# entn-at/exemplars_vc

Measured on AMD Instinct MI355X. Metric: spectral frames/sec converted (100 NMF iters, N=4096 dict), higher is better.
Workload: dtype f64

## Files before the change

exemplars_vc_amd/csrc/evc_fused_all.hip:

```cpp
#include "evc_fused_common.h"

namespace evc {

constexpr int AW = 4;
constexpr int AKT = 8;
constexpr int ATILES = AW * AKT;
constexpr int ATHREADS = 2 * AW * 64;
constexpr unsigned ALL_POLL_LIMIT = 1u << 17;
#ifndef EVC_ALL_STAGGER_PER_ITER
#define EVC_ALL_STAGGER_PER_ITER 11000
#endif
#ifndef EVC_ALL_EXCH_PRIO
#define EVC_ALL_EXCH_PRIO 3
#endif
#ifndef EVC_ALL_C1_ALTERNATE
#define EVC_ALL_C1_ALTERNATE 0
#endif

#ifdef EVC_ALL_TIMING
#define EVC_STAMP(i)                                                                                             \
    do {                                                                                                         \
        if (a.dbg && tt0 == g - half && lane == 0 && w == 0)                                                     \
            a.dbg[(((long)blockIdx.x * 2 + half) * (2 * a.iters + 1) + step) * 4 + (i)] = __builtin_amdgcn_s_memtime(); \
    } while (0)
#else
#define EVC_STAMP(i)
#endif

template <int MSTEPS, int C, bool KL>
__global__ __launch_bounds__(ATHREADS, 2) void k_fused_all(FusedArgs a) {
    constexpr int MT = MSTEPS > 4 ? 2 : 1;
    constexpr int E = MT * 4 * 64;
    constexpr int NE = MSTEPS * 64;
    constexpr int MSP = (MSTEPS + 1) & ~1;
    __shared__ double s_red[2][AW * E];
    __shared__ double s_v[2][E];
    __shared__ double s_x[2][E];
    __shared__ double s_r[2][KL ? E : 1];
    __shared__ double s_stage[2][C > 0 ? 1 : 768];
    __shared__ unsigned s_hb[2];
    __shared__ int s_fail;
    const int tid = threadIdx.x, lane = tid & 63;
    const int w8 = __builtin_amdgcn_readfirstlane(tid >> 6);
    const int half = w8 >> 2, w = w8 & 3, th = tid & (AW * 64 - 1);
    const int CR = C > 0 ? C : a.coop_c;
    const int member = blockIdx.x % CR;
    const int g = 2 * (blockIdx.x / CR) + half;
    double* const red = s_red[half];
    double* const vL = s_v[half];
    double* const xL = s_x[half];
    double* const rL = s_r[half];
    double* const stage = s_stage[half];
    unsigned hb = 0;
    const double* __restrict__ A1p = a.A1p;
    const double* __restrict__ A2p = a.A2p;
    f64x2* __restrict__ Hp = a.Hp;
    const int NT = a.NT;
    const long tile0 = (long)member * ATILES + w;
    const unsigned ul = (unsigned)lane;
    long sw = 0;

    const __amdgpu_buffer_rsrc_t r1 = __builtin_amdgcn_make_buffer_rsrc(const_cast<double*>(A1p), 0, NT * (MSP * 512), 0x00020000);
    const __amdgpu_buffer_rsrc_t r2 = __builtin_amdgcn_make_buffer_rsrc(const_cast<double*>(A2p), 0, NT * (MT * 2048), 0x00020000);
#ifdef EVC_ALL_NOFRAG
    bool nofrag_go = false;
#endif
    const unsigned ul16 = ul * 16u, ul8 = ul * 8u;
    auto load_a1 = [&](double (&a1)[MSTEPS], int k) {
#ifdef EVC_ALL_NOFRAG
        if (nofrag_go) return;
#endif
        const int so = (int)(tile0 + sw + AW * k) * (MSP * 512);
#pragma unroll
        for (int s = 0; s < MSTEPS; s += 2) {
            if (s + 1 < MSTEPS) {
                const f64x2 v = __builtin_bit_cast(f64x2, __builtin_amdgcn_raw_buffer_load_b128(r1, ul16 + (s >> 1) * 1024, so, 0));
                a1[s] = v[0];
                a1[s + 1] = v[1];
            } else {
                a1[s] = __builtin_bit_cast(double, __builtin_amdgcn_raw_buffer_load_b64(r1, ul16 + (s >> 1) * 1024, so, 0));
            }
        }
    };
    auto load_a2 = [&](double (&a2)[MT][4], int k) {
#ifdef EVC_ALL_NOFRAG
        if (nofrag_go) return;
#endif
        const int so = (int)(tile0 + sw + AW * k) * (MT * 2048);
#pragma unroll
        for (int u = 0; u < MT; ++u)
#pragma unroll
            for (int r = 0; r < 4; r += 2) {
                const f64x2 v = __builtin_bit_cast(f64x2, __builtin_amdgcn_raw_buffer_load_b128(r2, ul16 + (u * 2 + (r >> 1)) * 1024, so, 0));
                a2[u][r] = v[0];
                a2[u][r + 1] = v[1];
            }
    };
    (void)ul8;

    const int mode = a.eps_mode;
    const double eps = a.eps;
    const double d0 = a.l1 + (mode == EVC_EPS_ADD ? a.eps : 0.0);
    const f64x4 dinit = {d0, d0, d0, d0};
    const unsigned lo = fast_lo(mode, eps);
    unsigned seq = 0;
    int rs_es = 1, rs_len = 0, rs_pub0 = 0, rs_pub1 = 0, rs_src0 = -1, rs_src1 = -1, rs_src2 = -1;
    if (C < 0) {
        rs_es = (NE + CR - 1) / CR;
        rs_len = NE - member * rs_es;
        rs_len = rs_len < 0 ? 0 : (rs_len > rs_es ? rs_es : rs_len);
        const int e0 = th, e1 = th + AW * 64;
        const int j0 = e0 / rs_es, j1 = (e1 < NE ? e1 : e0) / rs_es;
        rs_pub0 = (j0 * CR + member) * rs_es + (e0 - j0 * rs_es);
        rs_pub1 = (j1 * CR + member) * rs_es + ((e1 < NE ? e1 : e0) - j1 * rs_es);
        auto src = [&](int idx) {
            if (idx >= CR * rs_es) return -1;
            const int el = idx % rs_es;
            return el < rs_len ? member * CR * rs_es + idx : -1;
        };
        rs_src0 = src(th);
        rs_src1 = src(th + AW * 64);
        rs_src2 = src(th + 2 * AW * 64);
    }
    if (tid == 0) s_fail = 0;
    if (tid < 2) s_hb[tid] = 0;

    if (a.stagger_cycles > 0 && ((blockIdx.x / CR) & 1)) {
        const long long t0 = __builtin_amdgcn_s_memtime();
        while (__builtin_amdgcn_s_memtime() - t0 < a.stagger_cycles) __builtin_amdgcn_s_sleep(32);
    }

    for (long tt0 = g - half; tt0 < a.TT; tt0 += a.groups) {
        const long tt = tt0 + half;
        bool valid;
        {
            const long t = 16 * tt + (lane & 15);
            int u = -1;
            if (tt < a.TT && t < a.T_) u = a.frame_utt[t];
            const bool live = tt < a.TT && ((t >= a.T_) || ((u >= 0) && (a.active[u] != 0)));
            const int v0 = __syncthreads_and(half == 0 ? live : true);
            const int v1 = __syncthreads_and(half == 1 ? live : true);
            valid = (half ? v1 : v0) != 0;
        }
        HTile h[AKT];
        f64x4 p[AKT];
        double a1[MSTEPS], a2[MT][4];
        if (valid && a.first && a.init_const) {
            auto h0_of = [&](int fr) {
                const long t = 16 * tt + fr;
                const int u = t < a.T_ ? a.frame_utt[t] : -1;
                return u >= 0 ? a.h0[u] : 0.0;
            };
            for (int e = th; e < E; e += AW * 64) {
                const int s = e >> 6, l = e & 63;
                const bool in = s < MSTEPS;
                xL[e] = in ? a.Xp[(tt * MSTEPS + s) * 64 + l] : 0.0;
                vL[e] = in ? a.rsum[bin_of(s, l >> 4)] * h0_of(l & 15) : 0.0;
                if (KL) rL[e] = xL[e] / (vL[e] < a.eps ? a.eps : vL[e]);
            }
            const double hv = h0_of(lane & 15);
#pragma unroll
            for (int k = 0; k < AKT; ++k) {
                const long n0 = 16 * (tile0 + AW * k) + 4 * (lane >> 4);
#pragma unroll
                for (int r = 0; r < 4; ++r) h[k][r] = n0 + r < a.N ? hv : 0.0;
            }
        } else if (valid) {
            for (int e = th; e < E; e += AW * 64) {
                const int s = e >> 6, l = e & 63;
                const bool in = s < MSTEPS;
                xL[e] = in ? a.Xp[(tt * MSTEPS + s) * 64 + l] : 0.0;
                vL[e] = in ? a.Vp[(tt * 8 + s) * 64 + l] : 0.0;
                if (KL) rL[e] = xL[e] / (vL[e] < a.eps ? a.eps : vL[e]);
            }
#pragma unroll
            for (int k = 0; k < AKT; ++k) {
                const f64x2* t = Hp + (tt * NT + tile0 + AW * k) * 128;
                const f64x2 h01 = t[ul], h23 = t[ul + 64];
                h[k][0] = h01[0]; h[k][1] = h01[1]; h[k][2] = h23[0]; h[k][3] = h23[1];
            }
        }
        __syncthreads();
        if (valid && !KL) {
            double x[MSTEPS];
#pragma unroll
            for (int s = 0; s < MSTEPS; ++s) x[s] = xL[s * 64 + lane];
            load_a1(a1, 0);
#pragma unroll
            for (int k = 0; k < AKT; ++k) {
                f64x4 acc = {0, 0, 0, 0};
#pragma unroll
                for (int s = 0; s < MSTEPS; ++s) acc = Mma<double>::mma(a1[s], x[s], acc);
                load_a1(a1, (k + 1) % AKT);
                p[k] = acc;
            }
        }

        if (valid && KL) load_a1(a1, 0);
        for (int step = 0; step <= 2 * a.iters; ++step) {
#ifdef EVC_ALL_NOFRAG
            nofrag_go = step > 2;
#endif
            const bool mine = (C == 1 && !EVC_ALL_C1_ALTERNATE) ? (step & 1) == 0 : (step & 1) == half;
            EVC_STAMP(0);
            if (valid && mine && step < 2 * a.iters) {
                asm volatile("" : "+s"(sw));
                double v[MSTEPS];
#pragma unroll
                for (int s = 0; s < MSTEPS; ++s) v[s] = KL ? rL[s * 64 + lane] : vL[s * 64 + lane];
                f64x4 vn[MT];
#pragma unroll
                for (int u = 0; u < MT; ++u) vn[u] = f64x4{0, 0, 0, 0};
#pragma unroll
                for (int k = 0; k < AKT; ++k) {
                    __builtin_amdgcn_sched_barrier(0);
                    load_a2(a2, k);
                    f64x4 d = KL ? f64x4{0, 0, 0, 0} : dinit;
#pragma unroll
                    for (int s = 0; s < MSTEPS; ++s) d = Mma<double>::mma(a1[s], v[s], d);
                    load_a1(a1, (k + 1) % AKT);
                    __builtin_amdgcn_sched_barrier(0);
                    if (KL) {
#pragma unroll
                        for (int r = 0; r < 4; ++r) h[k][r] *= d[r];
                    } else {
                        mu_tile_guarded(h[k], p[k], d, mode, eps, lo);
                    }
#pragma unroll
                    for (int u = 0; u < MT; ++u)
#pragma unroll
                        for (int r = 0; r < 4; ++r) vn[u] = Mma<double>::mma(a2[u][r], h[k][r], vn[u]);
                }
#pragma unroll
                for (int u = 0; u < MT; ++u)
#pragma unroll
                    for (int r = 0; r < 4; ++r)
                        if (u * 4 + r < MSTEPS) red[w * E + (u * 4 + r) * 64 + lane] = vn[u][r];
            } else if (valid && !mine && step > 0) {
                const int e0 = C <= 0 ? th % NE : th, e1 = th + AW * 64;
                const bool has1 = e1 < NE;
                __builtin_amdgcn_s_setprio(EVC_ALL_EXCH_PRIO);
                double s0 = 0.0, s1 = 0.0;
#pragma unroll
                for (int ww = 0; ww < AW; ++ww) {
                    s0 += red[ww * E + e0];
                    s1 += red[ww * E + (has1 ? e1 : e0)];
                }
                if (C < 0) {
                    long long* xb1 = reinterpret_cast<long long*>(a.coop_buf) +
                                     ((size_t)(seq & 1) * a.groups + g) * (size_t)CR * ALL_RS_STRIDE;
                    long long* xb2 = reinterpret_cast<long long*>(a.coop_buf) + ALL_SLICE_OFFSET +
                                     ((size_t)(seq & 1) * a.groups + g) * 512;
                    const long long tag = (seq >> 1) & 1;
                    __hip_atomic_store(xb1 + rs_pub0, (__double_as_longlong(s0) & ~1LL) | tag, __ATOMIC_RELAXED,
                                       __HIP_MEMORY_SCOPE_AGENT);
                    if (has1)
                        __hip_atomic_store(xb1 + rs_pub1, (__double_as_longlong(s1) & ~1LL) | tag, __ATOMIC_RELAXED,
                                           __HIP_MEMORY_SCOPE_AGENT);
                    bool ok = true;
                    auto fetch3 = [&](const long long* p0, const long long* p1, const long long* p2, long long& b0,
                                      long long& b1, long long& b2) {
                        unsigned polls = 0;
                        for (;;) {
                            b0 = __hip_atomic_load(p0, __ATOMIC_RELAXED, __HIP_MEMORY_SCOPE_AGENT);
                            b1 = __hip_atomic_load(p1, __ATOMIC_RELAXED, __HIP_MEMORY_SCOPE_AGENT);
                            b2 = __hip_atomic_load(p2, __ATOMIC_RELAXED, __HIP_MEMORY_SCOPE_AGENT);
                            if (__all(!ok || (((b0 ^ tag) | (b1 ^ tag) | (b2 ^ tag)) & 1) == 0)) break;
                            if (++polls > ALL_POLL_LIMIT ||
                                ((polls & 63) == 0 &&
                                 __hip_atomic_load(a.coop_abort, __ATOMIC_RELAXED, __HIP_MEMORY_SCOPE_AGENT) != 0))
                                ok = false;
                            __builtin_amdgcn_s_sleep(1);
                        }
                    };
                    {
                        long long b0, b1, b2;
                        const long long* own = xb1 + rs_pub0;
                        fetch3(rs_src0 >= 0 ? xb1 + rs_src0 : own, rs_src1 >= 0 ? xb1 + rs_src1 : own,
                               rs_src2 >= 0 ? xb1 + rs_src2 : own, b0, b1, b2);
                        if (rs_src0 >= 0) stage[th] = __longlong_as_double(b0 & ~1LL);
                        if (rs_src1 >= 0) stage[th + AW * 64] = __longlong_as_double(b1 & ~1LL);
                        if (rs_src2 >= 0) stage[th + 2 * AW * 64] = __longlong_as_double(b2 & ~1LL);
                        hb += AW;
                        if (lane == 0)
                            __hip_atomic_fetch_add(&s_hb[half], 1u, __ATOMIC_RELEASE, __HIP_MEMORY_SCOPE_WORKGROUP);
                        while ((int)(__hip_atomic_load(&s_hb[half], __ATOMIC_ACQUIRE, __HIP_MEMORY_SCOPE_WORKGROUP) - hb) < 0)
                            __builtin_amdgcn_s_sleep(1);
                        const int q = th & 3;
                        for (int el = th >> 2; el < rs_len; el += AW * 16) {
                            double v = 0.0;
                            for (int m = q; m < CR; m += 4) v += stage[m * rs_es + el];
                            v += __shfl_xor(v, 1, 64);
                            v += __shfl_xor(v, 2, 64);
                            if (q == 0)
                                __hip_atomic_store(xb2 + member * rs_es + el, (__double_as_longlong(v) & ~1LL) | tag,
                                                   __ATOMIC_RELAXED, __HIP_MEMORY_SCOPE_AGENT);
                        }
                    }
                    long long g0, g1, g2;
                    fetch3(xb2 + e0, xb2 + (has1 ? e1 : e0), xb2 + e0, g0, g1, g2);
                    s0 = __longlong_as_double(g0 & ~1LL);
                    s1 = __longlong_as_double(g1 & ~1LL);
                    ++seq;
                    if (!ok) s_fail = 1;
                } else if (C == 0) {
                    const int ES = NE / CR;
                    long long* xb1 = reinterpret_cast<long long*>(a.coop_buf) +
                                     ((size_t)(seq & 1) * a.groups + g) * (size_t)CR * 512;
                    long long* xb2 = reinterpret_cast<long long*>(a.coop_buf) + ALL_SLICE_OFFSET +
                                     ((size_t)(seq & 1) * a.groups + g) * 512;
                    const long long tag = (seq >> 1) & 1;
                    {
                        const int j0 = e0 / ES, j1 = (has1 ? e1 : e0) / ES;
                        __hip_atomic_store(xb1 + ((size_t)j0 * CR + member) * ES + (e0 - j0 * ES),
                                           (__double_as_longlong(s0) & ~1LL) | tag, __ATOMIC_RELAXED,
                                           __HIP_MEMORY_SCOPE_AGENT);
                        if (has1)
                            __hip_atomic_store(xb1 + ((size_t)j1 * CR + member) * ES + (e1 - j1 * ES),
                                               (__double_as_longlong(s1) & ~1LL) | tag, __ATOMIC_RELAXED,
                                               __HIP_MEMORY_SCOPE_AGENT);
                    }
                    bool ok = true;
                    auto fetch2 = [&](const long long* p0, const long long* p1, long long& b0, long long& b1) {
                        unsigned polls = 0;
                        for (;;) {
                            b0 = __hip_atomic_load(p0, __ATOMIC_RELAXED, __HIP_MEMORY_SCOPE_AGENT);
                            b1 = __hip_atomic_load(p1, __ATOMIC_RELAXED, __HIP_MEMORY_SCOPE_AGENT);
                            if (__all(!ok || (((b0 ^ tag) | (b1 ^ tag)) & 1) == 0)) break;
                            if (++polls > ALL_POLL_LIMIT ||
                                ((polls & 63) == 0 &&
                                 __hip_atomic_load(a.coop_abort, __ATOMIC_RELAXED, __HIP_MEMORY_SCOPE_AGENT) != 0))
                                ok = false;
                            __builtin_amdgcn_s_sleep(1);
                        }
                    };
                    {
                        long long b0, b1;
                        const long long* mine_ = xb1 + (size_t)member * NE;
                        fetch2(mine_ + e0, mine_ + (has1 ? e1 : e0), b0, b1);
                        stage[e0] = __longlong_as_double(b0 & ~1LL);
                        if (has1) stage[e1] = __longlong_as_double(b1 & ~1LL);
                        hb += AW;
                        if (lane == 0)
                            __hip_atomic_fetch_add(&s_hb[half], 1u, __ATOMIC_RELEASE, __HIP_MEMORY_SCOPE_WORKGROUP);
                        while ((int)(__hip_atomic_load(&s_hb[half], __ATOMIC_ACQUIRE, __HIP_MEMORY_SCOPE_WORKGROUP) - hb) < 0)
                            __builtin_amdgcn_s_sleep(1);
                        if (th < 4 * ES) {
                            const int el = th >> 2, q = th & 3, per = CR >> 2;
                            double v = 0.0;
                            for (int i = 0; i < per; ++i) v += stage[(q * per + i) * ES + el];
                            v += __shfl_xor(v, 1, 64);
                            v += __shfl_xor(v, 2, 64);
                            if (q == 0)
                                __hip_atomic_store(xb2 + member * ES + el, (__double_as_longlong(v) & ~1LL) | tag,
                                                   __ATOMIC_RELAXED, __HIP_MEMORY_SCOPE_AGENT);
                        }
                    }
                    long long g0, g1;
                    fetch2(xb2 + e0, xb2 + (has1 ? e1 : e0), g0, g1);
                    s0 = __longlong_as_double(g0 & ~1LL);
                    s1 = __longlong_as_double(g1 & ~1LL);
                    ++seq;
                    if (!ok) s_fail = 1;
                } else if (C > 1) {
                    long long* xb = reinterpret_cast<long long*>(a.coop_buf) +
                                    ((size_t)(seq & 1) * a.groups + g) * (size_t)(C * 512);
                    const long long tag = (seq >> 1) & 1;
                    const long long m0 = (__double_as_longlong(s0) & ~1LL) | tag;
                    const long long m1 = (__double_as_longlong(s1) & ~1LL) | tag;
                    __hip_atomic_store(xb + member * 512 + e0, m0, __ATOMIC_RELAXED, __HIP_MEMORY_SCOPE_AGENT);
                    if (has1) __hip_atomic_store(xb + member * 512 + e1, m1, __ATOMIC_RELAXED, __HIP_MEMORY_SCOPE_AGENT);
                    bool ok = true;
                    unsigned polls = 0;
                    {
                        const long long* sp = xb + (lane < C ? lane : 0) * 512 + (NE - 1);
                        for (;;) {
                            const long long b = __hip_atomic_load(sp, __ATOMIC_RELAXED, __HIP_MEMORY_SCOPE_AGENT);
                            const bool ready = lane >= C || lane == member || (b & 1) == tag;
                            if (__all(ready)) break;
                            if (++polls > ALL_POLL_LIMIT ||
                                ((polls & 63) == 0 &&
                                 __hip_atomic_load(a.coop_abort, __ATOMIC_RELAXED, __HIP_MEMORY_SCOPE_AGENT) != 0)) {
                                ok = false;
                                break;
                            }
                            __builtin_amdgcn_s_sleep(2);
                        }
                    }
                    long long b0[C > 0 ? C : 1] = {}, b1[C > 0 ? C : 1] = {};
                    polls = 0;
                    while (ok) {
#pragma unroll
                        for (int m = 0; m < C; ++m)
                            b0[m] = __hip_atomic_load(xb + m * 512 + e0, __ATOMIC_RELAXED, __HIP_MEMORY_SCOPE_AGENT);
#pragma unroll
                        for (int m = 0; m < C; ++m)
                            b1[m] = __hip_atomic_load(xb + m * 512 + (has1 ? e1 : e0), __ATOMIC_RELAXED, __HIP_MEMORY_SCOPE_AGENT);
                        long long bad = 0;
#pragma unroll
                        for (int m = 0; m < C; ++m) {
                            b0[m] = (m == member) ? m0 : b0[m];
                            b1[m] = (m == member) ? m1 : b1[m];
                            bad |= (b0[m] ^ tag) | (b1[m] ^ tag);
                        }
                        if ((bad & 1) == 0) break;
                        if (++polls > ALL_POLL_LIMIT ||
                            ((polls & 63) == 0 &&
                             __hip_atomic_load(a.coop_abort, __ATOMIC_RELAXED, __HIP_MEMORY_SCOPE_AGENT) != 0)) {
                            ok = false;
                            break;
                        }
                        __builtin_amdgcn_s_sleep(2);
                    }
                    s0 = 0.0; s1 = 0.0;
#pragma unroll
                    for (int m = 0; m < C; ++m) {
                        s0 += __longlong_as_double(b0[m] & ~1LL);
                        s1 += __longlong_as_double(b1[m] & ~1LL);
                    }
                    ++seq;
                    if (!ok) s_fail = 1;
                }
                vL[e0] = s0;
                if (has1) vL[e1] = s1;
                if (KL) {
                    rL[e0] = xL[e0] / (s0 < a.eps ? a.eps : s0);
                    if (has1) rL[e1] = xL[e1] / (s1 < a.eps ? a.eps : s1);
                }
                __builtin_amdgcn_s_setprio(0);
            }
            EVC_STAMP(1);
            __syncthreads();
            EVC_STAMP(2);
            if (C != 1 && s_fail) {
                if (tid == 0) __hip_atomic_store(a.coop_abort, 1, __ATOMIC_RELAXED, __HIP_MEMORY_SCOPE_AGENT);
                return;
            }
        }

        if (valid) {
#pragma unroll
            for (int k = 0; k < AKT; ++k) {
                f64x2* t = Hp + (tt * NT + tile0 + AW * k) * 128;
                t[ul] = f64x2{h[k][0], h[k][1]};
                t[ul + 64] = f64x2{h[k][2], h[k][3]};
            }
            if (a.Hx) {
                const long t = 16 * tt + (lane & 15);
                if (t < a.T_) {
#pragma unroll
                    for (int k = 0; k < AKT; ++k) {
                        const long n0 = 16 * (tile0 + AW * k) + 4 * (lane >> 4);
#pragma unroll
                        for (int r = 0; r < 4; ++r)
                            if (n0 + r < a.N) {
                                if (a.hx_frame_major) a.Hx[t * a.ldhx + n0 + r] = h[k][r];
                                else a.Hx[(n0 + r) * a.ldhx + t] = h[k][r];
                            }
                    }
                }
            }
            if (member == 0) {
                for (int e = th; e < NE; e += AW * 64) a.Vp[(tt * 8 + (e >> 6)) * 64 + (e & 63)] = vL[e];
                if (a.write_err && w == 0) {
                    double e = 0.0;
#pragma unroll
                    for (int s = 0; s < MSTEPS; ++s) {
                        const double x = xL[s * 64 + lane], vv = vL[s * 64 + lane];
                        e += KL ? kl_terms(x, vv, a.eps) : (x - vv) * (x - vv);
                    }
                    e += __shfl_xor(e, 16, 64);
                    e += __shfl_xor(e, 32, 64);
                    const long t = 16 * tt + lane;
                    if (lane < 16 && t < a.T_) a.err2[t] = e;
                }
            }
        }
        __syncthreads();
    }
}

template <int MSTEPS, int C, bool KL>
static hipError_t launch_all(FusedArgs a, int n_cus, hipStream_t s) {
    int occ = 0;
    hipError_t e = hipOccupancyMaxActiveBlocksPerMultiprocessor(&occ, k_fused_all<MSTEPS, C, KL>, ATHREADS, 0);
    if (e != hipSuccess) return e;
    if (occ < 1) return hipErrorInvalidValue;
    long resident = n_cus;
    if (2 * resident > ALL_MAX_WGS) resident = ALL_MAX_WGS / 2;
    const int cr = C > 0 ? C : a.coop_c;
    if (C == 0 && (cr < 8 || cr > 64 || (cr & (cr - 1)))) return hipErrorInvalidValue;
    if (C < 0 && (cr < 2 || cr > ALL_MAX_MEMBERS)) return hipErrorInvalidValue;
    int pairs = (int)(resident / cr);
    const int want = (a.TT + 1) / 2;
    if (pairs > want) pairs = want;
    if (pairs < 1) return hipErrorInvalidValue;
    a.groups = 2 * pairs;
    a.stagger_cycles = (a.iters > 0 && a.iters <= 25 && a.TT >= 4L * a.groups && pairs >= 2) ? (long long)a.iters * EVC_ALL_STAGGER_PER_ITER : 0;
    if (C != 1) {
        e = hipMemsetAsync(a.coop_buf, 0xFF, sizeof(double) * 2 * (size_t)a.groups * cr * (C < 0 ? ALL_RS_STRIDE : 512), s);
        if (e != hipSuccess) return e;
    }
    if (C <= 0) {
        if (2L * a.groups * 512 > ALL_SLICE_ELEMS) return hipErrorInvalidValue;
        e = hipMemsetAsync(a.coop_buf + ALL_SLICE_OFFSET, 0xFF, sizeof(double) * 2 * (size_t)a.groups * 512, s);
        if (e != hipSuccess) return e;
    }
    hipLaunchKernelGGL((k_fused_all<MSTEPS, C, KL>), dim3((unsigned)(pairs * cr)), dim3(ATHREADS), 0, s, a);
    return hipGetLastError();
}

template <int MSTEPS, bool KL>
static hipError_t pick_c(const FusedArgs& a, int n_cus, hipStream_t s) {
    switch (a.NT / ATILES) {
        case 1: return launch_all<MSTEPS, 1, KL>(a, n_cus, s);
        case 2: return launch_all<MSTEPS, 2, KL>(a, n_cus, s);
        case 4: return launch_all<MSTEPS, 4, KL>(a, n_cus, s);
#ifdef EVC_ALL_DIRECT8
        case 8: return launch_all<MSTEPS, 8, KL>(a, n_cus, s);
#else
        case 8:
#endif
        case 16:
        case 32:
        case 64: return launch_all<MSTEPS, 0, KL>(a, n_cus, s);
        default: return launch_all<MSTEPS, -1, KL>(a, n_cus, s);
    }
}

int fused_all_members(int NT, int N, int eps_mode, int exact_div, int loss) {
    if (eps_mode == EVC_EPS_NONE || exact_div || (loss != EVC_LOSS_FROBENIUS && loss != EVC_LOSS_KL)) return 0;
    if (NT % ATILES) return 0;
    const int c = NT / ATILES;
    if (loss == EVC_LOSS_KL && c >= 2 && c < 16) return 0;
    return (c >= 1 && c <= ALL_MAX_MEMBERS) ? c : 0;
}

hipError_t fused_all_launch(int msteps, const FusedArgs& a, int n_cus, hipStream_t s) {
    if (a.NT % ATILES || !a.coop_buf || !a.coop_abort) return hipErrorInvalidValue;
    switch (msteps) {
        case 1: return a.loss == EVC_LOSS_KL ? pick_c<1, true>(a, n_cus, s) : pick_c<1, false>(a, n_cus, s);
        case 2: return a.loss == EVC_LOSS_KL ? pick_c<2, true>(a, n_cus, s) : pick_c<2, false>(a, n_cus, s);
        case 3: return a.loss == EVC_LOSS_KL ? pick_c<3, true>(a, n_cus, s) : pick_c<3, false>(a, n_cus, s);
        case 4: return a.loss == EVC_LOSS_KL ? pick_c<4, true>(a, n_cus, s) : pick_c<4, false>(a, n_cus, s);
        case 5: return a.loss == EVC_LOSS_KL ? pick_c<5, true>(a, n_cus, s) : pick_c<5, false>(a, n_cus, s);
        case 6: return a.loss == EVC_LOSS_KL ? pick_c<6, true>(a, n_cus, s) : pick_c<6, false>(a, n_cus, s);
        case 7: return a.loss == EVC_LOSS_KL ? pick_c<7, true>(a, n_cus, s) : pick_c<7, false>(a, n_cus, s);
        case 8: return a.loss == EVC_LOSS_KL ? pick_c<8, true>(a, n_cus, s) : pick_c<8, false>(a, n_cus, s);
        default: return hipErrorInvalidValue;
    }
}

}
```

Baseline: 1.052 million.

## Keep each workgroup's dictionary slice resident in LDS instead of reloading from global

When it fits in the LDS budget and the loss is Frobenius, each workgroup copies its dictionary tiles once into shared memory in a padded, row-permuted layout. Both matrix-product phases then read the A1/A2 fragments from LDS instead of issuing buffer loads from global memory on every NMF iteration. The 8-member case is routed to a direct C=8 instantiation when the dictionary fits. This adds LDS pressure, which may lower occupancy, adds a one-time fill cost, and sizes the reduction and staging buffers from compile-time shape constants.

Result: faster. 1.095 million (median of 6 runs) (+4.1%).

```diff
diff --git a/exemplars_vc_amd/csrc/evc_fused_all.hip b/exemplars_vc_amd/csrc/evc_fused_all.hip
--- a/exemplars_vc_amd/csrc/evc_fused_all.hip
+++ b/exemplars_vc_amd/csrc/evc_fused_all.hip
@@ -16,6 +16,25 @@
 #ifndef EVC_ALL_C1_ALTERNATE
 #define EVC_ALL_C1_ALTERNATE 0
 #endif
+
+constexpr long ALL_LDS_BUDGET = 160 * 1024 - 256;
+__host__ __device__ constexpr int all_dict_row(int e) { return 4 * (((e >> 2) & 1) * 2 + (e >> 3)) + (e & 3); }
+template <int MSTEPS, int C, bool KL>
+struct AllShape {
+    static constexpr int MT = MSTEPS > 4 ? 2 : 1;
+    static constexpr int E = MT * 4 * 64;
+    static constexpr int NE = MSTEPS * 64;
+    static constexpr int RSTR = NE < 256 ? 256 : NE;
+    static constexpr int STG = C > 0 ? 1 : (C == 0 ? NE : NE + ALL_MAX_MEMBERS - 1);
+    static constexpr long REST = 8L * 2 * (AW * RSTR + 2 * E + (KL ? E : 1) + STG) + 3 * 4;
+    static constexpr long dict_bytes(int pr) { return 8L * ATILES * 16 * pr; }
+    static constexpr int PR_ALL = 4 * MSTEPS + 2;
+    static constexpr int PR = KL ? 0
+                              : REST + dict_bytes(PR_ALL) <= ALL_LDS_BUDGET       ? PR_ALL
+                              : REST + dict_bytes(PR_ALL - 4) <= ALL_LDS_BUDGET   ? PR_ALL - 4
+                                                                                  : 0;
+    static constexpr bool LDS_DICT = C != 1 && PR > 0 && PR - 1 >= 4 * MSTEPS - 3;
+};
 
 #ifdef EVC_ALL_TIMING
 #define EVC_STAMP(i)                                                                                             \
@@ -29,15 +48,20 @@
 
 template <int MSTEPS, int C, bool KL>
 __global__ __launch_bounds__(ATHREADS, 2) void k_fused_all(FusedArgs a) {
-    constexpr int MT = MSTEPS > 4 ? 2 : 1;
-    constexpr int E = MT * 4 * 64;
-    constexpr int NE = MSTEPS * 64;
+    using S = AllShape<MSTEPS, C, KL>;
+    constexpr int MT = S::MT;
+    constexpr int E = S::E;
+    constexpr int NE = S::NE;
+    constexpr int RSTR = S::RSTR;
     constexpr int MSP = (MSTEPS + 1) & ~1;
-    __shared__ double s_red[2][AW * E];
+    constexpr int PR = S::PR;
+    constexpr int TPD = 16 * PR;
+    __shared__ double s_red[2][AW * RSTR];
     __shared__ double s_v[2][E];
     __shared__ double s_x[2][E];
     __shared__ double s_r[2][KL ? E : 1];
-    __shared__ double s_stage[2][C > 0 ? 1 : 768];
+    __shared__ double s_stage[2][S::STG];
+    __shared__ double s_dict[S::LDS_DICT ? ATILES * TPD : 1];
     __shared__ unsigned s_hb[2];
     __shared__ int s_fail;
     const int tid = threadIdx.x, lane = tid & 63;
@@ -66,7 +90,23 @@
     bool nofrag_go = false;
 #endif
     const unsigned ul16 = ul * 16u, ul8 = ul * 8u;
-    auto load_a1 = [&](double (&a1)[MSTEPS], int k) {
+    constexpr int BL = 16 * ((MSTEPS - 1) >> 2) + 4 * ((MSTEPS - 1) & 3);
+    const int rowA = w * AKT * TPD + all_dict_row(4 * (lane & 3) + ((lane & 15) >> 2)) * PR;
+    const int rowB = w * AKT * TPD + all_dict_row(4 * (lane >> 4)) * PR;
+    const double* const dA = s_dict + rowA + (lane >> 4);
+    const double* const dAL = s_dict + rowA + min(lane >> 4, a.M - BL);
+    const double* const dB = s_dict + rowB + (lane & 15);
+    const double* const dBL = s_dict + rowB + min(lane & 15, a.M - 16 * (MT - 1));
+#define LDS_NO_PAIR() asm volatile("" ::: "memory")
+    auto load_a1 = [&](double (&a1)[MSTEPS], int k, auto lds) {
+        if constexpr (decltype(lds)::value) {
+#pragma unroll
+            for (int s = 0; s < MSTEPS; ++s) {
+                a1[s] = (s == MSTEPS - 1 ? dAL : dA)[k * TPD + 16 * (s >> 2) + 4 * (s & 3)];
+                LDS_NO_PAIR();
+            }
+            return;
+        }
 #ifdef EVC_ALL_NOFRAG
         if (nofrag_go) return;
 #endif
@@ -82,7 +122,17 @@
             }
         }
     };
-    auto load_a2 = [&](double (&a2)[MT][4], int k) {
+    auto load_a2 = [&](double (&a2)[MT][4], int k, auto lds) {
+        if constexpr (decltype(lds)::value) {
+#pragma unroll
+            for (int u = 0; u < MT; ++u)
+#pragma unroll
+                for (int r = 0; r < 4; ++r) {
+                    a2[u][r] = (u == MT - 1 ? dBL : dB)[k * TPD + r * PR + 16 * u];
+                    LDS_NO_PAIR();
+                }
+            return;
+        }
 #ifdef EVC_ALL_NOFRAG
         if (nofrag_go) return;
 #endif
@@ -130,6 +180,7 @@
         while (__builtin_amdgcn_s_memtime() - t0 < a.stagger_cycles) __builtin_amdgcn_s_sleep(32);
     }
 
+    auto run = [&](auto lds) __attribute__((always_inline)) {
     for (long tt0 = g - half; tt0 < a.TT; tt0 += a.groups) {
         const long tt = tt0 + half;
         bool valid;
@@ -185,18 +236,18 @@
             double x[MSTEPS];
 #pragma unroll
             for (int s = 0; s < MSTEPS; ++s) x[s] = xL[s * 64 + lane];
-            load_a1(a1, 0);
+            load_a1(a1, 0, lds);
 #pragma unroll
             for (int k = 0; k < AKT; ++k) {
                 f64x4 acc = {0, 0, 0, 0};
 #pragma unroll
                 for (int s = 0; s < MSTEPS; ++s) acc = Mma<double>::mma(a1[s], x[s], acc);
-                load_a1(a1, (k + 1) % AKT);
+                if (!decltype(lds)::value || k + 1 < AKT) load_a1(a1, (k + 1) % AKT, lds);
                 p[k] = acc;
             }
         }
 
-        if (valid && KL) load_a1(a1, 0);
+        if (valid && KL) load_a1(a1, 0, lds);
         for (int step = 0; step <= 2 * a.iters; ++step) {
 #ifdef EVC_ALL_NOFRAG
             nofrag_go = step > 2;
@@ -208,17 +259,19 @@
                 double v[MSTEPS];
 #pragma unroll
                 for (int s = 0; s < MSTEPS; ++s) v[s] = KL ? rL[s * 64 + lane] : vL[s * 64 + lane];
+                if constexpr (decltype(lds)::value) load_a1(a1, 0, lds);
                 f64x4 vn[MT];
 #pragma unroll
                 for (int u = 0; u < MT; ++u) vn[u] = f64x4{0, 0, 0, 0};
 #pragma unroll
                 for (int k = 0; k < AKT; ++k) {
                     __builtin_amdgcn_sched_barrier(0);
-                    load_a2(a2, k);
+                    load_a2(a2, k, lds);
                     f64x4 d = KL ? f64x4{0, 0, 0, 0} : dinit;
 #pragma unroll
                     for (int s = 0; s < MSTEPS; ++s) d = Mma<double>::mma(a1[s], v[s], d);
-                    load_a1(a1, (k + 1) % AKT);
+                    if (!decltype(lds)::value || k + 1 < AKT)
+                        load_a1(a1, (k + 1) % AKT, lds);
                     __builtin_amdgcn_sched_barrier(0);
                     if (KL) {
 #pragma unroll
@@ -235,7 +288,7 @@
                 for (int u = 0; u < MT; ++u)
 #pragma unroll
                     for (int r = 0; r < 4; ++r)
-                        if (u * 4 + r < MSTEPS) red[w * E + (u * 4 + r) * 64 + lane] = vn[u][r];
+                        if (u * 4 + r < MSTEPS) red[w * RSTR + (u * 4 + r) * 64 + lane] = vn[u][r];
             } else if (valid && !mine && step > 0) {
                 const int e0 = C <= 0 ? th % NE : th, e1 = th + AW * 64;
                 const bool has1 = e1 < NE;
@@ -243,8 +296,8 @@
                 double s0 = 0.0, s1 = 0.0;
 #pragma unroll
                 for (int ww = 0; ww < AW; ++ww) {
-                    s0 += red[ww * E + e0];
-                    s1 += red[ww * E + (has1 ? e1 : e0)];
+                    s0 += red[ww * RSTR + e0];
+                    s1 += red[ww * RSTR + (has1 ? e1 : e0)];
                 }
                 if (C < 0) {
                     long long* xb1 = reinterpret_cast<long long*>(a.coop_buf) +
@@ -478,6 +531,22 @@
         }
         __syncthreads();
     }
+    };
+
+    if constexpr (S::LDS_DICT) {
+        if (a.M > 0 && a.M < PR) {
+            for (int x = tid; x < ATILES * TPD; x += ATHREADS) {
+                const int slot = x / TPD, e = all_dict_row((x / PR) % 16), b = x % PR;
+                const long j = (long)member * ATILES + slot / AKT + AW * (slot % AKT);
+                const int q = e >> 2, r = e & 3;
+                s_dict[x] = b < a.M ? A2p[((j * MT + (b >> 4)) * 2 + (r >> 1)) * 128 + (16 * q + (b & 15)) * 2 + (r & 1)] : 0.0;
+            }
+            __syncthreads();
+            run(std::true_type{});
+            return;
+        }
+    }
+    run(std::false_type{});
 }
 
 template <int MSTEPS, int C, bool KL>
@@ -516,11 +585,10 @@
         case 1: return launch_all<MSTEPS, 1, KL>(a, n_cus, s);
         case 2: return launch_all<MSTEPS, 2, KL>(a, n_cus, s);
         case 4: return launch_all<MSTEPS, 4, KL>(a, n_cus, s);
-#ifdef EVC_ALL_DIRECT8
-        case 8: return launch_all<MSTEPS, 8, KL>(a, n_cus, s);
-#else
         case 8:
-#endif
+            if constexpr (AllShape<MSTEPS, 8, KL>::LDS_DICT)
+                if (a.M > 0 && a.M < AllShape<MSTEPS, 8, KL>::PR) return launch_all<MSTEPS, 8, KL>(a, n_cus, s);
+            return launch_all<MSTEPS, 0, KL>(a, n_cus, s);
         case 16:
         case 32:
         case 64: return launch_all<MSTEPS, 0, KL>(a, n_cus, s);
```
